# FedeMont/collision_handling_in_instantNGP

Measured on AMD Instinct MI355X. Metric: Mpixels/sec fwd+bwd at L=16,F=2,T=2^19, higher is better.
Workload: dtype f32

## Files before the change

collision_handling_in_instantngp_amd/_lib.py:

```python
import ctypes
import os

import torch

_HERE = os.path.dirname(os.path.abspath(__file__))
LIB_PATH = os.environ.get("GNGF_LIB_PATH") or os.path.join(_HERE, "libgngf_hip.so")

_c = ctypes
_P = _c.c_void_p
_I = _c.c_int
_L = _c.c_int64
_F = _c.c_float
_D = _c.c_double

SIGNATURES = {
    "gngf_abi_version": [],
    "gngf_hash_indices": [_P, _P, _P, _L, _I, _L, _P],
    "gngf_mrhe_fwd": [_P, _I, _P, _P, _P, _L, _I, _I, _L, _I, _I, _P],
    "gngf_mrhe_bwd": [_P, _I, _P, _P, _P, _P, _P, _L, _I, _I, _L, _I, _I, _P],
    "gngf_bilinear_fwd": [_P, _P, _P, _P, _L, _I, _I, _P],
    "gngf_bilinear_bwd": [_P, _P, _P, _P, _L, _I, _I, _P],
    "gngf_encode_fwd": [_P, _P, _I, _P, _P, _P, _P, _L, _I, _I, _L, _I, _I, _I, _L, _I, _I, _P, _P],
    "gngf_encode_bwd": [_P, _P, _I, _P, _P, _P, _P, _P, _P, _L, _I, _I, _L, _I, _I, _I, _L, _I, _I, _P],
    "gngf_encode_bwd_bucketed_plan": [_L, _I, _L, _I, _I, _P],
# ... 86 lines not shown
    "gngf_ext2_version": [],
    "gngf_ext2_render_score_workspace_words": [],
    "gngf_ext2_render_score": [_P, _I, _P, _P, _P, _P, _P, _P, _P, _P, _P, _I, _I, _L, _I, _I, _I, _L, _I, _I,
                               _P, _L, _L, _I, _F, _L, _P, _P, _P],
}

EXT2_VERSION = 1

_QUERY_TAIL = [_P, _L, _P, _P, _P]
EXT3_SIGNATURES = {
    "gngf_ext3_version": [],
    "gngf_ext3_query": [_P, _I, _P, _P, _P, _P, _P, _P, _P, _P, _P, _I, _I, _L, _I, _I, _I, _L, _I, _I] + _QUERY_TAIL,
    "gngf_ext3_query_grid": [_P, _P, _P, _P, _P, _P, _P, _P, _P, _I, _I, _I, _I] + _QUERY_TAIL,
    "gngf_ext3_vertex_grid_bwd_flat_owned": list(SIGNATURES["gngf_vertex_grid_bwd_flat"]),
    "gngf_ext3_encode_tiled_bwd_clear_rows": SIGNATURES["gngf_encode_tiled_bwd"][:-1] + [_P, _P, _I, _P],
}

EXT3_VERSION = 2

EXT3_WRITES_NOTHING = {
    "gngf_ext3_version": "returns a constant",
}


class BinJob(ctypes.Structure):
    _fields_ = [("xy", _P), ("P", _L), ("tile_shift", _I), ("NB", _I), ("chunk", _I), ("blockhist", _P), ("persistent_ws", _P),
                ("tile_off", _P), ("tile_item_base", _P), ("items", _P), ("n_items", _P), ("sorted", _P)]


_RETURNS_INT64 = {"gngf_decoder_hidden_floats", "gngf_slot_bitmap_words"}
_lib = None


class GngfLibraryError(RuntimeError):
    pass


def load():
    global _lib
    if _lib is not None:
        return _lib
    if not os.path.isfile(LIB_PATH):
        raise GngfLibraryError(
            f"{LIB_PATH} not found: build it with `python -c 'import __graft_entry__ as g; g.build()'` "
            "or `make -C collision_handling_in_instantngp_amd/csrc`.  There is no CPU fallback.")
    lib = ctypes.CDLL(LIB_PATH)
    for name, argtypes in (list(SIGNATURES.items()) + list(EXT_SIGNATURES.items()) + list(EXT2_SIGNATURES.items())
                           + list(EXT3_SIGNATURES.items())):
        try:
            fn = getattr(lib, name)
        except AttributeError as e:
            raise GngfLibraryError(f"{LIB_PATH} does not export {name}: stale build?") from e
        fn.argtypes = argtypes
        fn.restype = _L if name in _RETURNS_INT64 else _I
    ver = lib.gngf_abi_version()
    if ver != ABI_VERSION:
        raise GngfLibraryError(f"ABI version mismatch: library {ver}, binding {ABI_VERSION}")
    ext = lib.gngf_ext_version()
    if ext != EXT_VERSION:
        raise GngfLibraryError(f"extension version mismatch (include/gngf_ext.h): library {ext}, binding {EXT_VERSION}")
    ext2 = lib.gngf_ext2_version()
    if ext2 != EXT2_VERSION:
        raise GngfLibraryError(f"extension version mismatch (include/gngf_ext2.h): library {ext2}, binding {EXT2_VERSION}")
    ext3 = lib.gngf_ext3_version()
    if ext3 != EXT3_VERSION:
        raise GngfLibraryError(f"extension version mismatch (include/gngf_ext3.h): library {ext3}, binding {EXT3_VERSION}")
    _lib = lib
    return lib


def stream_ptr():
    return _P(torch.cuda.current_stream().cuda_stream)


def ptr(t, dtype=None, name="tensor"):
    if t is None:
        return _P(0)
    if not t.is_cuda:
        raise GngfLibraryError(f"{name} is on {t.device}: the gfx950 path needs CUDA/HIP tensors (no CPU fallback)")
    if dtype is not None and t.dtype != dtype:
        raise TypeError(f"{name} must be {dtype}, got {t.dtype}")
    if not t.is_contiguous():
        raise ValueError(f"{name} must be contiguous")
    return _P(t.data_ptr())


def query(name, *args):
    return getattr(load(), name)(*args)

# ... 17 lines not shown
```

collision_handling_in_instantngp_amd/csrc/decoder.hip:

```cpp
#include "gngf_common.h"
#include <type_traits>
#include <utility>

#include "decoder_common.inc"

namespace gngf {

__device__ __forceinline__ float vmax0(float z) { float r; asm("v_max_f32 %0, 0, %1" : "=v"(r) : "v"(z)); return r; }
template <bool LEAKY> __device__ __forceinline__ float hidden_act(float z) {
  if (LEAKY) { float r; const float t = 0.01f * z; asm("v_max_f32 %0, %1, %2" : "=v"(r) : "v"(z), "v"(t)); return r; }
  return vmax0(z);
}
template <bool LEAKY> __device__ __forceinline__ float hidden_dsel(float y, float d) { return y > 0.f ? d : (LEAKY ? 0.01f * d : 0.f); }

using f32x2 = __attribute__((ext_vector_type(2))) float;
__device__ __forceinline__ unsigned lds_addr(const float* p) {
  return (unsigned)(size_t)(__attribute__((address_space(3))) const float*)p;
}
template <int OFF> __device__ __forceinline__ void lds_store(unsigned addr, float v) {
  static_assert(OFF >= 0 && OFF < 65536, "ds offset is 16 bits");
  asm volatile("ds_write_b32 %0, %1 offset:%2" : : "v"(addr), "v"(v), "n"(OFF) : "memory");
}
template <int OFF> __device__ __forceinline__ f32x2 lds_load2(unsigned addr) {
  static_assert(OFF >= 0 && OFF < 65536, "ds offset is 16 bits");
// ... 29 lines not shown
  static constexpr int kA0 = 2 * S0 * 64, kA1 = 2 * 32 * 64, kA2 = 32 * 64;
};

template <int KIN>
__device__ __forceinline__ void fill_fwd_frags(float* A0, float* A1, const float* raw, int in_dim) {
  constexpr int S0 = KIN / 2;
  const RawOff o = raw_offsets(in_dim);
  for (int e = threadIdx.x; e < 2 * S0 * 64; e += kDecThreads) {
    const int lane = e & 63, s = (e >> 6) % S0, t = (e >> 6) / S0;
    const int i = lane & 31, h = lane >> 5, k = h * S0 + s;
    A0[e] = k < in_dim ? raw[o.w0 + (32 * t + i) * (in_dim + 1) + k] : 0.f;
  }
  for (int e = threadIdx.x; e < 2 * 32 * 64; e += kDecThreads) {
    const int lane = e & 63, s2 = (e >> 6) & 31, t = e >> 11;
    const int i = lane & 31, h = lane >> 5;
    A1[e] = raw[o.w1 + (32 * t + i) * 65 + kmapC(s2, h)];
  }
}

using u32x4 = __attribute__((ext_vector_type(4))) unsigned;

__device__ unsigned long long g_bwd_span[2];

#if defined(GNGF_STAMPS)
__device__ unsigned long long g_stamps[16];
__device__ unsigned long long g_fstamps[16];
__device__ unsigned long long g_blocktime[2][256][2];
#ifndef GNGF_STAMP_MASK
#define GNGF_STAMP_MASK 0xffff
#endif
#define STAMP(k) do { if constexpr ((((GNGF_STAMP_MASK) >> (k)) & 1) != 0) { unsigned long long t_; __builtin_amdgcn_sched_barrier(0); \
    asm volatile("s_memtime %0\n\ts_waitcnt lgkmcnt(0)" : "=s"(t_) :: "memory"); __builtin_amdgcn_sched_barrier(0); \
    ph[k] += t_ - tlast; tlast = t_; } } while (0)
#else
#define STAMP(k) do {} while (0)
#endif

constexpr int kHiddenTileFloats = 2 * 4 * 8 * 64 * 4;
#ifndef GNGF_BWD_X_AUX
#define GNGF_BWD_X_AUX 0
#endif
#ifndef GNGF_HIDDEN_AUX
#define GNGF_HIDDEN_AUX 2
#endif
#ifndef GNGF_HIDDEN_ST_AUX
#define GNGF_HIDDEN_ST_AUX GNGF_HIDDEN_AUX
// ... 173 lines not shown
    for (int k = 0; k < 10; ++k) g_fstamps[k] = ph[k];
  if (threadIdx.x == 0) g_blocktime[0][blockIdx.x & 255][1] = __builtin_readcyclecounter();
#endif
}

__host__ __device__ inline int slab_sums(int in_dim, int out_dim) { return kH * in_dim + kH * kH + out_dim * kH + 2 * kH + out_dim; }
__host__ __device__ inline int slab_size(int in_dim, int out_dim) { return slab_sums(in_dim, out_dim) + 1; }

constexpr int kImgStride = 34;
constexpr int kImgFloats = 64 * kImgStride;
#include "decoder_split.inc"
template <int KIN> struct BwdLds {
  static constexpr bool kDedicatedX = KIN <= 32;
  static constexpr int kWaveFloats = 2 * kImgFloats + 4 * kImgStride + (kDedicatedX ? KIN * kImgStride : 0);
};

template <int KIN, bool LEAKY, bool EXACT, bool RECOMPUTE, bool HYB = false, bool TRAIN = false>
__global__ void __launch_bounds__(kDecThreads, 1)
decoder_bwd_kernel(const float* __restrict__ X, const float* __restrict__ Yout, const float* __restrict__ dY,
                   const float* __restrict__ W0, const float* __restrict__ b0, const float* __restrict__ W1,
                   const float* __restrict__ b1, const float* __restrict__ W2, float* __restrict__ dX,
                   float* __restrict__ slabs, const float* __restrict__ hidden, int64_t P, int in_dim, int out_dim,
                   const float* __restrict__ target, const float* __restrict__ gloss, const float* __restrict__ b2 = nullptr,
                   float4* __restrict__ zero_fill = nullptr, int64_t zero_vecs = 0) {
  using FF = FwdFrags<KIN>;
  constexpr int S0 = KIN / 2;
  constexpr int TX = (KIN + 31) / 32;
  if (EXACT) in_dim = KIN;
  if (blockIdx.x == 0 && threadIdx.x == 0) { g_bwd_span[1] = 0ull; g_bwd_span[0] = wall_clock64(); }
#if defined(GNGF_STAMPS)
  if (threadIdx.x == 0) g_blocktime[1][blockIdx.x & 255][0] = __builtin_readcyclecounter();
#endif
  extern __shared__ float smem[];
  float* A0 = smem;
  float* A1 = A0 + FF::kA0;
  float* A2T = A1 + FF::kA1;
  static_assert(!HYB || (KIN == 32 && EXACT && !RECOMPUTE), "hybrid variant: 32 input features, saved hidden layers");
  static_assert(!TRAIN || HYB, "the fused training kernel builds on the hybrid backward");
  constexpr int kA1T = HYB ? 8 * 3 * 64 * 4 : 2 * 32 * 64, kA0T = HYB ? 4 * 3 * 64 * 4 : TX * 32 * 64;
  float* A1T = A2T + 2 * 2 * 64;
  float* A0T = A1T + kA1T;
  float* bs = A0T + kA0T;
  float* img = bs + 2 * kH;
  const int nslab = slab_size(in_dim, out_dim);

  float* raw = img;
  stage_raw(raw, W0, b0, W1, b1, W2, TRAIN ? b2 : nullptr, in_dim, out_dim);
// ... 134 lines not shown
    const __amdgpu_buffer_rsrc_t ry = __builtin_amdgcn_make_buffer_rsrc(const_cast<float*>(Yout) + tt * 128 * out_dim, 0, rows * out_dim * 4, 0x00020000);
    const __amdgpu_buffer_rsrc_t rd = __builtin_amdgcn_make_buffer_rsrc(const_cast<float*>(dsrc) + tt * 128 * out_dim, 0, rows * out_dim * 4, 0x00020000);
    if constexpr (TRAIN) {
#pragma unroll
      for (int sk = 0; sk < 2; ++sk) dyn[sk] = __uint_as_float(__builtin_amdgcn_raw_buffer_load_b32(rd, yoffh[sk], 0, 0));
    } else {
#pragma unroll
    for (int c = 0; c < 4; ++c) {
      const unsigned off = c < out_dim ? yoff + 4u * c : 0x40000000u;
      yn[c] = __uint_as_float(__builtin_amdgcn_raw_buffer_load_b32(ry, off, 0, 0));
      dyn[c] = __uint_as_float(__builtin_amdgcn_raw_buffer_load_b32(rd, off, 0, 0));
    }
    }
  };
  auto make_dz3 = [&]() {
#pragma unroll
    for (int c = 0; c < (TRAIN ? 2 : 4); ++c) {
      const float dy = fused_loss ? kloss * (yn[c] - dyn[c]) : dyn[c];
      dz3[c] = dy * (yn[c] * (1.f - yn[c]));
      asm volatile("" : "+v"(dz3[c]));
      db2acc[c] += dz3[c];
    }
  };
  fetch_x(blockIdx.x);
  fetch_y(blockIdx.x);
  if constexpr (!TRAIN) make_dz3();
  float b2v[4] = {0.f, 0.f, 0.f, 0.f};
  if constexpr (TRAIN) {
#pragma unroll
    for (int sk = 0; sk < 2; ++sk) b2v[sk] = raw[ro.b2 + 2 * sk + h];
  }
  f32x16 b0v[2], b1v[2];
  if (RECOMPUTE) {
#pragma unroll
    for (int t = 0; t < 2; ++t) {
#pragma unroll
      for (int r = 0; r < 16; ++r) { b0v[t][r] = bs[32 * t + crow(r, h)]; b1v[t][r] = bs[kH + 32 * t + crow(r, h)]; }
      asm volatile("" : "+a"(b0v[t]), "+a"(b1v[t]));
    }
  }
  unsigned dxmax = 0u;
#if defined(GNGF_STAMPS)
  unsigned ph[16] = {0, 0, 0, 0, 0, 0, 0, 0, 0, 0, 0, 0, 0, 0, 0, 0};
  unsigned long long tlast;
  asm volatile("s_memtime %0\n\ts_waitcnt lgkmcnt(0)" : "=s"(tlast) :: "memory");
#endif
// ... 20 lines not shown
  };
  if constexpr (HYB && !TRAIN) static_for<16>([&](auto E) { store_hidden_images(E); });
  const u32x4* w1t = reinterpret_cast<const u32x4*>(A1T) + lane;
  const u32x4* w0t = reinterpret_cast<const u32x4*>(A0T) + lane;
  Planes w1p[HYB ? 8 : 1], w0p[HYB ? 4 : 1];
  if constexpr (HYB) {
#pragma unroll
    for (int f = 0; f < 8; ++f) {
      w1p[f] = load_planes(w1t + f * 3 * 64);
      asm volatile("" : "+a"(w1p[f].hi), "+a"(w1p[f].mid), "+a"(w1p[f].lo));
    }
  }
  u32x4* w1f = reinterpret_cast<u32x4*>(A1T);
  if constexpr (TRAIN) {
    asm volatile("s_waitcnt lgkmcnt(0)" ::: "memory");
    __syncthreads();
    for (int f = threadIdx.x >> 6; f < 8; f += 4) {
      const int cc = f >> 1, t = f & 1;
      const float* r1 = raw + ro.w1 + (32 * t + i) * 65;
      store_planes(w1f + f * 3 * 64 + lane, split8(r1[kmapS(cc, h, 0)], r1[kmapS(cc, h, 1)], r1[kmapS(cc, h, 2)], r1[kmapS(cc, h, 3)],
                                                  r1[kmapS(cc, h, 4)], r1[kmapS(cc, h, 5)], r1[kmapS(cc, h, 6)], r1[kmapS(cc, h, 7)]));
    }
    __syncthreads();
  }
  if (RECOMPUTE && kCarryF0) {
#pragma unroll
    for (int sx = 0; sx < S0; ++sx) { f0[0][sx] = A0[(0 * S0 + sx) * 64 + lane]; f0[1][sx] = A0[(1 * S0 + sx) * 64 + lane]; }
  }
#define STEP_END() __builtin_amdgcn_sched_barrier(0)
#define SLOT_END() __builtin_amdgcn_sched_barrier(0)
#define SLOT_END1(x) do { asm volatile("" : "+a"(x)); __builtin_amdgcn_sched_barrier(0); } while (0)
#define SLOT_END2(x, y) do { asm volatile("" : "+a"(x), "+a"(y)); __builtin_amdgcn_sched_barrier(0); } while (0)
  for (int64_t tile = blockIdx.x; tile < ntiles; tile += gridDim.x) {
    pin_acc();
    STAMP(0);
    float f1[2][32];
    float a2t[2][2];
    if constexpr (TRAIN) {
      Planes pa0 = load_planes(w0f + lane), pa1 = load_planes(w0f + 3 * 64 + lane);
#pragma unroll
      for (int t = 0; t < 2; ++t)
#pragma unroll
        for (int g = 0; g < 4; ++g) {
          const f32x4 q0 = *reinterpret_cast<const f32x4*>(bs + 32 * t + 8 * g + 4 * h);
          const f32x4 q1 = *reinterpret_cast<const f32x4*>(bs + kH + 32 * t + 8 * g + 4 * h);
#pragma unroll
          for (int e = 0; e < 4; ++e) { acc1[t][4 * g + e] = q0[e]; acc2[t][4 * g + e] = q1[e]; }
        }
      Planes zc = split8(xr[0], xr[1], xr[2], xr[3], xr[4], xr[5], xr[6], xr[7]);
      STAMP(8);
      unsigned nh[4], nm[4], nl[4];
      float sra, srb;
      auto next_planes = [&]() {
        Planes p;
        p.hi = u32x4{nh[0], nh[1], nh[2], nh[3]}; p.mid = u32x4{nm[0], nm[1], nm[2], nm[3]}; p.lo = u32x4{nl[0], nl[1], nl[2], nl[3]};
        return p;
      };
// ... 165 lines not shown
        if constexpr (TRAIN) {
          fa[0][sk] = a2t[0][sk]; fa[1][sk] = a2t[1][sk];
          bsel[sk] = dz3[sk];
        } else {
        fa[0][sk] = A2T[(0 * 2 + sk) * 64 + lane]; fa[1][sk] = A2T[(1 * 2 + sk) * 64 + lane];
        float lo = dz3[2 * sk], hi = dz3[2 * sk + 1];
        asm volatile("" : "+v"(lo), "+v"(hi));
        bsel[sk] = h == 0 ? lo : hi;
        }
      }
      STEP_END();
      MFMA_VV_ZERO(d2[0], fa[0][0], bsel[0]); MFMA_VV_ZERO(d2[1], fa[1][0], bsel[0]);
      MFMA_VV(d2[0], fa[0][1], bsel[1]); MFMA_VV(d2[1], fa[1][1], bsel[1]);
      if constexpr (TRAIN) {
        asm volatile("" : "+v"(d2[0]), "+v"(d2[1]));
        STEP_END();
      }
      if constexpr (!RECOMPUTE) {
        if (BL::kDedicatedX) static_for<S0>([&](auto SX) { lds_store<kImgX + SX.value * kImgStride * 4>(wX, xr[SX.value]); });
        if constexpr (TRAIN) static_for<2>([&](auto SK) { lds_store<kImgZ + 2 * SK.value * kImgStride * 4>(wDz3h, dz3[SK.value]); });
        else static_for<4>([&](auto C) { lds_store<kImgZ + C.value * kImgStride * 4>(wDz3, dz3[C.value]); });
      }
    }
    if (!RECOMPUTE && BL::kDedicatedX) fetch_x(tile + gridDim.x);
    fetch_y(tile + gridDim.x);
    MFMA_DRAIN(d2[0], d2[1]);
    STEP_END();
    STAMP(12);
    if constexpr (TRAIN) {
#pragma unroll
      for (int r = 0; r < 8; ++r) d2[0][r] = hidden_dsel<LEAKY>(acc2[0][r], d2[0][r]);
    } else {
#pragma unroll
    for (int t = 0; t < 2; ++t)
#pragma unroll
      for (int r = 0; r < 16; ++r) {
        if (RECOMPUTE) acc2[t][r] = hidden_act<LEAKY>(acc2[t][r]);
        d2[t][r] = hidden_dsel<LEAKY>(acc2[t][r], d2[t][r]);
      }
    }
    pin_acc();
    STEP_END();
    STAMP(3);
    f32x16 d1[2];
    f32x2 a0p[8], a1p[8], b0p[8], b1p[8];
    float h1v[2][16];
    if constexpr (HYB) {
      f32x2 av[16], bv[16];
// ... 355 lines not shown
          const int col = 32 * tx + 8 * g + 4 * h;
          if (EXACT) {
            if (32 * tx + 8 * g + 8 <= KIN) {
              u32x4 v = {__float_as_uint(dxv[tx][4 * g]), __float_as_uint(dxv[tx][4 * g + 1]), __float_as_uint(dxv[tx][4 * g + 2]),
                         __float_as_uint(dxv[tx][4 * g + 3])};
              __builtin_amdgcn_raw_buffer_store_b128(v, rs, base + 4u * col, 0, 0);
            }
          } else {
#pragma unroll
            for (int q = 0; q < 4; ++q)
              __builtin_amdgcn_raw_buffer_store_b32(__float_as_uint(dxv[tx][4 * g + q]), rs, col + q < in_dim ? base + 4u * (col + q) : 0x40000000u, 0, 0);
          }
        }
    }
    if constexpr (kClears) {
      for (int z = 0; z < zper; ++z, zlo += kDecThreads)
        if (zlo < zhi) zero_fill[zlo] = float4{0.f, 0.f, 0.f, 0.f};
    }
    pin_acc();
    STEP_END();
    STAMP(7);
  }

#if defined(GNGF_STAMPS)
  if (blockIdx.x == 7 && threadIdx.x == 0)
    for (int k = 0; k < 16; ++k) g_stamps[k] = ph[k];
  if (threadIdx.x == 0) g_blocktime[1][blockIdx.x & 255][1] = __builtin_readcyclecounter();
#endif
#pragma unroll
  for (int o = 32; o > 0; o >>= 1) { const unsigned ov = (unsigned)__shfl_xor((int)dxmax, o, 64); dxmax = ov > dxmax ? ov : dxmax; }
  __syncthreads();
  float* region = smem + wave * nslab;
  float* sW0 = region;
  float* sW1 = sW0 + kH * in_dim;
  float* sW2 = sW1 + kH * kH;
  float* sb0 = sW2 + out_dim * kH;
  float* sb1 = sb0 + kH;
  float* sb2 = sb1 + kH;
#pragma unroll
  for (int ti = 0; ti < 2; ++ti)
#pragma unroll
    for (int r = 0; r < 16; ++r) {
      const int row = 32 * ti + crow(r, h);
#pragma unroll
      for (int tj = 0; tj < 2; ++tj) sW1[row * kH + 32 * tj + i] = dW1acc[ti][tj][r];
#pragma unroll
// ... 117 lines not shown
  GNGF_CHECK_ARG(slabs && (!reduce_here || (dW0 && db0 && dW1 && db1 && dW2 && db2)));
  const int nslab = slab_size(in_dim, out_dim);
  hipStream_t s = as_stream(stream);
  const int nslabs = gngf_decoder_bwd_slabs(P);
  if (P == 0) {
    hipError_t e = zero_async(slabs, sizeof(float) * (size_t)nslab, s);
    if (e != hipSuccess) return (int)e;
    if (zero_fill && zero_floats > 0) {
      e = zero_async(zero_fill, sizeof(float) * (size_t)zero_floats, s);
      if (e != hipSuccess) return (int)e;
    }
  } else {
    GNGF_CHECK_ARG(enc && rgb && (target ? gloss != nullptr : drgb != nullptr) && W0 && b0 && W1 && b1 && W2 && denc);
    if (zero_fill && zero_floats > 0 && in_dim != 64) {
      hipError_t e = zero_async(zero_fill, sizeof(float) * (size_t)zero_floats, s);
      if (e != hipSuccess) return (int)e;
    }
    if (g_decoder_bwd_hybrid && in_dim == 32 && hidden) {
      const size_t smem = bwd_smem_bytes_hybrid(out_dim);
      auto fn = leaky ? decoder_bwd_kernel<32, true, true, false, true> : decoder_bwd_kernel<32, false, true, false, true>;
      hipError_t e = hipFuncSetAttribute(reinterpret_cast<const void*>(fn), hipFuncAttributeMaxDynamicSharedMemorySize, (int)smem);
      if (e != hipSuccess) return (int)e;
      fn<<<dim3((unsigned)nslabs), dim3(kDecThreads), smem, s>>>(enc, rgb, drgb, W0, b0, W1, b1, W2, denc, slabs, hidden, P, in_dim, out_dim,
                                                                 target, gloss, nullptr, zf, zv);
    } else
    DISPATCH_KIN(in_dim, {
      const size_t smem = bwd_smem_bytes<kKIN>(in_dim, out_dim);
      using Kern = void (*)(const float*, const float*, const float*, const float*, const float*, const float*, const float*,
                            const float*, float*, float*, const float*, int64_t, int, int, const float*, const float*, const float*,
                            float4*, int64_t);
      const bool exact = in_dim == kKIN;
      Kern fn;
      if (hidden)
        fn = leaky ? (exact ? decoder_bwd_kernel<kKIN, true, true, false> : decoder_bwd_kernel<kKIN, true, false, false>)
                   : (exact ? decoder_bwd_kernel<kKIN, false, true, false> : decoder_bwd_kernel<kKIN, false, false, false>);
      else
        fn = leaky ? (exact ? decoder_bwd_kernel<kKIN, true, true, true> : decoder_bwd_kernel<kKIN, true, false, true>)
                   : (exact ? decoder_bwd_kernel<kKIN, false, true, true> : decoder_bwd_kernel<kKIN, false, false, true>);
      hipError_t e = hipFuncSetAttribute(reinterpret_cast<const void*>(fn), hipFuncAttributeMaxDynamicSharedMemorySize, (int)smem);
      if (e != hipSuccess) return (int)e;
      fn<<<dim3((unsigned)nslabs), dim3(kDecThreads), smem, s>>>(enc, rgb, drgb, W0, b0, W1, b1, W2, denc, slabs, hidden, P, in_dim, out_dim,
                                                                 target, gloss, nullptr, zf, zv);
    });
    hipError_t e = hipGetLastError();
    if (e != hipSuccess) return (int)e;
  }
  if (reduce_here)
    decoder_reduce_kernel<<<dim3((unsigned)((nslab + 63) / 64)), dim3(1024), 0, s>>>(slabs, nslabs, nslab, in_dim, out_dim, dW0,
                                                                                     db0, dW1, db1, dW2, db2, denc_absmax, nullptr, nullptr);
  GNGF_RETURN_LAUNCH();
}

extern "C" int gngf_decoder_train(const float* enc, const float* target, const float* gloss, const float* W0, const float* b0,
                                  const float* W1, const float* b1, const float* W2, const float* b2, float* rgb, float* denc,
                                  float* dW0, float* db0, float* dW1, float* db1, float* dW2, float* db2, float* slabs,
                                  float* denc_absmax, float* zero_fill, int64_t zero_floats, int64_t P, int in_dim, int out_dim,
                                  int leaky, void* stream) {
  GNGF_CHECK_ARG(P > 0 && in_dim == 32 && out_dim > 0 && out_dim <= 4);
  GNGF_CHECK_ARG(!zero_fill || (zero_floats >= 0 && (zero_floats & 3) == 0 && (reinterpret_cast<uintptr_t>(zero_fill) & 15) == 0));
  const bool reduce_here = dW0 || db0 || dW1 || db1 || dW2 || db2;
  GNGF_CHECK_ARG(slabs && (!reduce_here || (dW0 && db0 && dW1 && db1 && dW2 && db2)));
  GNGF_CHECK_ARG(enc && target && gloss && W0 && b0 && W1 && b1 && W2 && b2 && rgb && denc);
  const int nslab = slab_size(in_dim, out_dim);
  hipStream_t s = as_stream(stream);
  const int nslabs = gngf_decoder_bwd_slabs(P);
  const size_t smem = bwd_smem_bytes_hybrid(out_dim);
  auto fn = leaky ? decoder_bwd_kernel<32, true, true, false, true, true> : decoder_bwd_kernel<32, false, true, false, true, true>;
  hipError_t e = hipFuncSetAttribute(reinterpret_cast<const void*>(fn), hipFuncAttributeMaxDynamicSharedMemorySize, (int)smem);
  if (e != hipSuccess) return (int)e;
  fn<<<dim3((unsigned)nslabs), dim3(kDecThreads), smem, s>>>(enc, rgb, nullptr, W0, b0, W1, b1, W2, denc, slabs, nullptr, P, in_dim, out_dim,
                                                             target, gloss, b2, reinterpret_cast<float4*>(zero_fill),
                                                             zero_fill ? zero_floats / 4 : 0);
  e = hipGetLastError();
  if (e != hipSuccess) return (int)e;
  if (reduce_here)
    decoder_reduce_kernel<<<dim3((unsigned)((nslab + 63) / 64)), dim3(1024), 0, s>>>(slabs, nslabs, nslab, in_dim, out_dim, dW0,
                                                                                     db0, dW1, db1, dW2, db2, denc_absmax, nullptr, nullptr);
  GNGF_RETURN_LAUNCH();
}

extern "C" int gngf_decoder_reduce(const float* slabs, float* dW0, float* db0, float* dW1, float* db1, float* dW2, float* db2,
                                   float* denc_absmax, const float* gloss_promised, const float* gloss_arrived, int64_t P,
                                   int in_dim, int out_dim, void* stream) {
  GNGF_CHECK_ARG(P >= 0 && in_dim > 0 && in_dim <= 64 && out_dim > 0 && out_dim <= 4);
  GNGF_CHECK_ARG(slabs && dW0 && db0 && dW1 && db1 && dW2 && db2 && (!gloss_promised == !gloss_arrived));
  const int nslab = slab_size(in_dim, out_dim);
  decoder_reduce_kernel<<<dim3((unsigned)((nslab + 63) / 64)), dim3(1024), 0, as_stream(stream)>>>(
      slabs, gngf_decoder_bwd_slabs(P), nslab, in_dim, out_dim, dW0, db0, dW1, db1, dW2, db2, denc_absmax, gloss_promised,
      gloss_arrived);
  GNGF_RETURN_LAUNCH();
}

extern "C" int gngf_decoder_bwd_last_span_ns(double* ns) {
  GNGF_CHECK_ARG(ns);
  unsigned long long span[2] = {0ull, 0ull};
  hipError_t e = hipMemcpyFromSymbol(span, HIP_SYMBOL(gngf::g_bwd_span), sizeof(span));
  if (e != hipSuccess) return (int)e;
  *ns = span[1] > span[0] ? (double)(span[1] - span[0]) * 10.0 : 0.0;
  return 0;
}

#if defined(GNGF_STAMPS)
extern "C" int gngf_debug_read_fwd_stamps(unsigned long long* host16) {
  return (int)hipMemcpyFromSymbol(host16, HIP_SYMBOL(gngf::g_fstamps), 16 * sizeof(unsigned long long));
}
extern "C" int gngf_debug_read_blocktime(unsigned long long* host1024) {
  return (int)hipMemcpyFromSymbol(host1024, HIP_SYMBOL(gngf::g_blocktime), 2 * 256 * 2 * sizeof(unsigned long long));
}
extern "C" int gngf_debug_read_stamps(unsigned long long* host16) {
  return (int)hipMemcpyFromSymbol(host16, HIP_SYMBOL(gngf::g_stamps), 16 * sizeof(unsigned long long));
}
#endif

#include "render.inc"
```

collision_handling_in_instantngp_amd/ops.py:

```python
import ctypes as _ct
import dataclasses as _dc
import math as _math
import os
import sys as _sys
import types as _types

import torch

from . import _lib
from ._lib import call, ptr, query, stream_ptr

BLEND_CODES = {True: 0, None: 1, False: 2}
MODE_HASH, MODE_VERTEX_TABLE = 0, 1
MODE_DENSE_HASH = 2
MAX_TOPK = 128
MAX_TOPK_LIST = 32


def check_topk(K):
    K = int(K)
    if K > MAX_TOPK:
        raise ValueError(f"topk_k = {K} exceeds the limit of {MAX_TOPK} (ops.MAX_TOPK, GNGF_MAX_TOPK_WIDE)")
    return K

# ... 1268 lines not shown
    if not TUNING.use_side_stream:
        return torch.cuda.current_stream(device)
    key = (device.type, device.index, torch.cuda.current_stream(device).stream_id)
    if key not in _SIDE_STREAMS:
        _SIDE_STREAMS[key] = torch.cuda.Stream(device=device)
    return _SIDE_STREAMS[key]


@_dc.dataclass(frozen=True)
class StepConfig:
    source: str
    staged: int
    direct: int
    binning: str
    vertex_fwd: str
    pixel: str
    grad_sink: str
    table_grad: str
    clear: str
    direct_bwd: str
    exchange: bool
    vertex_bwd_flat: bool = False
    owned_rows: bool = False

    def signature(self):
        return (f"{self.source} L{self.staged}+{self.direct} bin={self.binning} vfwd={self.vertex_fwd} px={self.pixel} sink={self.grad_sink} "
                f"dE={self.table_grad}/{self.clear} direct={self.direct_bwd}" + (" xchg" if self.exchange else "")
                + (" vbwd=flat" if self.vertex_bwd_flat else "") + (" rows=owned" if self.owned_rows else ""))

    def chain(self):
        lv = ("tiled" if self.staged else "") + ("+" if self.staged and self.direct else "") + ("direct" if self.direct else "")
        return (f"{self.source} {lv} bin={self.binning} vfwd={self.vertex_fwd} px={self.pixel} sink={self.grad_sink} "
                f"dE={self.table_grad}/{self.clear} direct={self.direct_bwd}" + (" xchg" if self.exchange else ""))

    @staticmethod
    def choose(plan, L, T, F, P, mode, fp32_tables, needs_grad, link_defer_zero, link_zero_hidden, exchange, persist_ok, persist_alloc_ok,
               have_reserve_ws, flat_list=False, owned_rows=False):
        t = TUNING
        tiled = plan.Ls > 0 and P > 0
        nd = L - plan.Ls
        if mode == MODE_DENSE_HASH:
            if exchange:
                raise ValueError("the dense-where-it-fits index source does not run under a data-parallel exchange")
            dbw = "atomics" if (needs_grad and nd > 0) else "none"
            if not tiled:
                return StepConfig("dense_hash", 0, L, "none", "none", "none", "none", "alloc" if needs_grad else "none", "none", dbw, False)
            il = plan.interleaved(backward=bool(needs_grad))
            if not needs_grad:
                return StepConfig("dense_hash", plan.Ls, nd, "prepare", "riders", "interleaved" if il else "generic", "none", "none", "none",
                                  "none", False)
# ... 51 lines not shown
        K = check_topk(0 if vert_idx is None else vert_idx.shape[1])
        NV = 0 if vert_idx is None else vert_idx.shape[0]
        enc = torch.empty((P, L * F), dtype=_f32, device=tables.device)
        ws = None
        ctx.flat = (_flat_list_of(order, plan, vert_idx, vert_w, T)
                    if (P > 0 and ctx.needs_input_grad[3] and not ctx.needs_input_grad[5]) else None)
        if vert_idx is not None and order is None and plan.Ls > 0 and P > 0 and ctx.needs_input_grad[3]:
            order = slot_order(vert_idx, plan.n_ls_host[:plan.Ls], vstride)
        buf = None
        clear_now = None
        dev = tables.device
        tiled = plan.Ls > 0 and P > 0
        pws = _bin_workspace(dev, plan.ntiles, dp, kind="reserve") if (tiled and TUNING.fused_vertex_fwd) else None
        choose_args = (
            plan, L, T, F, P, mode, tables.dtype == _f32, bool(ctx.needs_input_grad[3]),
            bool(link is not None and link.defer_zero), bool(link is not None and link.zero_hidden),
            bool(dp is not None and dp.exchange is not None), bool(dp is not None and dp.persist_ok and getattr(dp, "level_params", None)),
            bool(dp is not None and (getattr(dp, "persist_grad", None) is not None or not torch.cuda.is_current_stream_capturing())),
            bool(pws is not None and pws.numel() >= 2 * plan.ntiles + 3))
        want_owned = bool(VERTEX_BWD_OWNED and ctx.flat is not None
                          and StepConfig.choose(*choose_args, flat_list=True, owned_rows=True).owned_rows)
        sc = ctx.step_config = StepConfig.choose(*choose_args, flat_list=ctx.flat is not None,
                                                 owned_rows=want_owned and _owned_peek(dp, tables, ctx.flat) is not None)
        if dp is not None:
            dp.step_config = sc
        _trace("step_config", signature=sc.signature())
        if SEEN_STEP_CONFIGS is not None:
            SEEN_STEP_CONFIGS.add(sc.chain())
        if tiled:
            fused = sc.vertex_fwd == "fused" and sc.binning == "pipeline"
            use64 = sc.grad_sink == "dG64"
            if ctx.needs_input_grad[3]:
                ng = 0 if sc.grad_sink == "table_rows" else ((plan.vtot * F + 2) * 2 if use64 else plan.vtot * F)
                nt = tables.numel()
                if fused and sc.owned_rows:
                    big = torch.empty(((ng + 3) & ~3,), dtype=_f32, device=dev)
                    buf = _BackwardBuffers(big[:ng].view(_i64), None, zbuf=big, owned=True)
                elif fused:
                    big = torch.empty((nt + ((ng + 3) & ~3),), dtype=_f32, device=dev)
                    dgrid = None if ng == 0 else (big[nt:nt + ng].view(_i64) if use64 else big[nt:nt + ng].view(plan.vtot, F))
                    buf = _BackwardBuffers(dgrid, big[:nt].view(tables.shape), zbuf=big)
                else:
                    dgrid = None if ng == 0 else (torch.empty((plan.vtot * F + 2,), dtype=_i64, device=dev) if use64
                                                  else torch.empty((plan.vtot, F), dtype=_f32, device=dev))
                    if sc.table_grad == "persist":
                        clear_now = _persistent_peek(dp, tables)
# ... 443 lines not shown
        return
    call("gngf_ext3_query", *pointers, *scalars, ptr(xy, _f32, "xy"), P, ptr(out_rgb, _f32, "out_rgb"),
         ptr(out_image, _i32, "out_image"), stream_ptr())


def query_grid_points(grid, n_ls, n_ls_host, decoder_params, xy, *, leaky=False, out_rgb=None, out_image=None):
    C, pointers, scalars = _grid_model("query_grid_points", grid, n_ls, n_ls_host, decoder_params, leaky)
    P = _query_tail("query_grid_points", xy, C, out_rgb, out_image)
    if P == 0:
        return
    call("gngf_ext3_query_grid", *pointers, *scalars, ptr(xy, _f32, "xy"), P, ptr(out_rgb, _f32, "out_rgb"),
         ptr(out_image, _i32, "out_image"), stream_ptr())



def _at_end_of_backward(fn):
    try:
        torch.autograd.Variable._execution_engine.queue_callback(fn)
    except RuntimeError:
        fn()


_GLOSS_SCALARS = {}


def _decoder_grad_buffers(ws, P, in_dim, out_dim, dev):
    flat = torch.empty((sum(w.numel() for w in ws),), dtype=_f32, device=dev)
    grads, off = [], 0
    for w in ws:
        grads.append(flat[off:off + w.numel()].view(w.shape))
        off += w.numel()
    nslabs, nslab = _lib.query("gngf_decoder_bwd_slabs", P), _lib.query("gngf_decoder_slab_floats", in_dim, out_dim)
    slabs = torch.empty((nslabs * nslab,), dtype=_f32, device=dev)
    return flat, grads, slabs, nslabs, nslab


def _decoder_fwd(ctx, enc, leaky, ws, target, gloss_known=None, link=None):
    ctx.ws_given = tuple(ws)
    ctx.link = link = link if link is not None else StepLink()
    enc = _c(enc)
    ws = [_c(w) for w in ws]
    P, in_dim = enc.shape
    out_dim = ws[4].shape[0]
    dev = enc.device
    rgb = torch.empty((P, out_dim), dtype=_f32, device=dev)
    hidden = None
    ctx.train = None
    train = (TUNING.decoder_train_fusion and gloss_known is not None and target is not None and in_dim == 32 and P > 0
             and TUNING.decoder_reduce_rides and any(ctx.needs_input_grad))
    if TUNING.decoder_save_hidden and P > 0 and any(ctx.needs_input_grad) and not train:
        hidden = torch.empty((_lib.query("gngf_decoder_hidden_floats", P),), dtype=_f32, device=dev)
    if target is not None:
        if P == 0:
            raise ValueError("MSE of an empty batch")
        target = _c(target)
        if tuple(target.shape) != (P, out_dim) or target.dtype != _f32:
            raise ValueError(f"target {tuple(target.shape)} / {target.dtype} does not match the decoder output ({P}, {out_dim}) float32")
    if train:
        key = (dev, float(gloss_known))
        gl = _GLOSS_SCALARS.get(key)
        if gl is None:
            if len(_GLOSS_SCALARS) > 64:
                _GLOSS_SCALARS.clear()
            gl = _GLOSS_SCALARS[key] = torch.full((), float(gloss_known), dtype=_f32, device=dev)
        target_c = _c(target)
        denc = torch.empty_like(enc)
        flat, grads, slabs, nslabs, nslab = _decoder_grad_buffers(ws, P, in_dim, out_dim, dev)
        zr, link.zero_request = link.zero_request, None
        call("gngf_decoder_train", ptr(enc, _f32, "enc"), ptr(target_c, _f32, "target"), ptr(gl), *[ptr(w, _f32) for w in ws], ptr(rgb),
             ptr(denc), *[ptr(None)] * 6, ptr(slabs), ptr(None), ptr(zr), 0 if zr is None else zr.numel(), P, in_dim, out_dim,
             int(leaky), stream_ptr())
        ctx.train = {"denc": denc, "flat": flat, "grads": grads, "slabs": slabs, "nslabs": nslabs, "nslab": nslab,
                     "gloss": float(gloss_known), "promised": gl}
    else:
        call("gngf_decoder_fwd", ptr(enc, _f32, "enc"), *[ptr(w, _f32) for w in ws], ptr(rgb), ptr(hidden), P, in_dim, out_dim, int(leaky),
             stream_ptr())
    mse = None
    if target is not None:
        wsp = _MSE_WORKSPACE.get(dev)
        if wsp is None:
            wsp = _MSE_WORKSPACE[dev] = torch.zeros(query("gngf_mse_workspace_floats"), dtype=_f32, device=dev)
        mse = torch.empty((), dtype=_f32, device=dev)
        if link.loss_value_aside:
            link.loss_value = {"pred": rgb, "label": target, "loss": mse, "ws": wsp, "device": dev,
                               "stream": torch.cuda.current_stream(dev).cuda_stream, "stream_obj": torch.cuda.current_stream(dev)}
        else:
            call("gngf_mse_fwd", ptr(rgb), ptr(target), ptr(mse), ptr(wsp), rgb.numel(), stream_ptr())
    ctx.save_for_backward(enc, rgb, target, *ws)
    ctx.hidden = hidden
    ctx.cfg = (P, in_dim, out_dim, int(leaky))
    return rgb, mse


def _grads_are_adopted(ctx):
# ... 160 lines not shown
```

Measured before the change: 2738.

## Add per-wave stagger option and incremental next-tile prefetch in decoder train kernel

Adds an optional per-wave sleep stagger after the prologue of the fused decoder train kernel, exposed through a new ext4 entry point, with a default of zero so the default path runs no sleeps. It also replaces the per-tile fetch_x/fetch_y prefetch in the forward (train) path with an incremental window pointer that advances by gridDim and builds buffer resources sized to the remaining rows. That is meant to cut 64-bit address arithmetic on each tile. A debug wave-phase timestamp probe is added behind a compile flag.

```diff
diff --git a/collision_handling_in_instantngp_amd/_lib.py b/collision_handling_in_instantngp_amd/_lib.py
--- a/collision_handling_in_instantngp_amd/_lib.py
+++ b/collision_handling_in_instantngp_amd/_lib.py
@@ -132,6 +132,28 @@
     "gngf_ext3_version": "returns a constant",
 }
 
+_U64 = ctypes.c_uint64
+EXT4_SIGNATURES = {
+    "gngf_ext4_version": [],
+    "gngf_ext4_decoder_train_default_stagger": [],
+    "gngf_ext4_decoder_train": SIGNATURES["gngf_decoder_train"][:-1] + [_U64, _P],
+}
+
+EXT4_VERSION = 1
+MAX_STAGGER_UNITS = 1023
+DEFAULT_DECODER_TRAIN_STAGGER = 0
+
+
+def stagger_pattern(l0, l1, l2, l3):
+    lags = (int(l0), int(l1), int(l2), int(l3))
+    if any(l < 0 or l > 0xffff for l in lags):
+        raise ValueError(f"stagger lags are 16-bit fields: {lags}")
+    return lags[0] | lags[1] << 16 | lags[2] << 32 | lags[3] << 48
+
+
+def stagger_lags(pattern):
+    return tuple((int(pattern) >> (16 * w)) & 0xffff for w in range(4))
+
 
 class BinJob(ctypes.Structure):
     _fields_ = [("xy", _P), ("P", _L), ("tile_shift", _I), ("NB", _I), ("chunk", _I), ("blockhist", _P), ("persistent_ws", _P),
@@ -139,6 +161,7 @@
 
 
 _RETURNS_INT64 = {"gngf_decoder_hidden_floats", "gngf_slot_bitmap_words"}
+_RETURNS_UINT64 = {"gngf_ext4_decoder_train_default_stagger"}
 _lib = None
 
 
@@ -156,13 +179,13 @@
             "or `make -C collision_handling_in_instantngp_amd/csrc`.  There is no CPU fallback.")
     lib = ctypes.CDLL(LIB_PATH)
     for name, argtypes in (list(SIGNATURES.items()) + list(EXT_SIGNATURES.items()) + list(EXT2_SIGNATURES.items())
-                           + list(EXT3_SIGNATURES.items())):
+                           + list(EXT3_SIGNATURES.items()) + list(EXT4_SIGNATURES.items())):
         try:
             fn = getattr(lib, name)
         except AttributeError as e:
             raise GngfLibraryError(f"{LIB_PATH} does not export {name}: stale build?") from e
         fn.argtypes = argtypes
-        fn.restype = _L if name in _RETURNS_INT64 else _I
+        fn.restype = _L if name in _RETURNS_INT64 else (_U64 if name in _RETURNS_UINT64 else _I)
     ver = lib.gngf_abi_version()
     if ver != ABI_VERSION:
         raise GngfLibraryError(f"ABI version mismatch: library {ver}, binding {ABI_VERSION}")
@@ -175,6 +198,13 @@
     ext3 = lib.gngf_ext3_version()
     if ext3 != EXT3_VERSION:
         raise GngfLibraryError(f"extension version mismatch (include/gngf_ext3.h): library {ext3}, binding {EXT3_VERSION}")
+    ext4 = lib.gngf_ext4_version()
+    if ext4 != EXT4_VERSION:
+        raise GngfLibraryError(f"extension version mismatch (include/gngf_ext4.h): library {ext4}, binding {EXT4_VERSION}")
+    stagger = lib.gngf_ext4_decoder_train_default_stagger()
+    if stagger != DEFAULT_DECODER_TRAIN_STAGGER:
+        raise GngfLibraryError(f"default stagger pattern mismatch (include/gngf_ext4.h): library {stagger:#x}, "
+                               f"binding {DEFAULT_DECODER_TRAIN_STAGGER:#x}")
     _lib = lib
     return lib
 
diff --git a/collision_handling_in_instantngp_amd/csrc/decoder.hip b/collision_handling_in_instantngp_amd/csrc/decoder.hip
--- a/collision_handling_in_instantngp_amd/csrc/decoder.hip
+++ b/collision_handling_in_instantngp_amd/csrc/decoder.hip
@@ -1,4 +1,5 @@
 #include "gngf_common.h"
+#include "../../include/gngf_ext4.h"
 #include <type_traits>
 #include <utility>
 
@@ -75,6 +76,10 @@
 
 __device__ unsigned long long g_bwd_span[2];
 
+#if defined(GNGF_WAVE_PHASE)
+constexpr int kPhaseTiles[5] = {0, 1, 8, 16, 31};
+__device__ unsigned g_wave_phase[4][4][5];
+#endif
 #if defined(GNGF_STAMPS)
 __device__ unsigned long long g_stamps[16];
 __device__ unsigned long long g_fstamps[16];
@@ -294,7 +299,7 @@
                    const float* __restrict__ b1, const float* __restrict__ W2, float* __restrict__ dX,
                    float* __restrict__ slabs, const float* __restrict__ hidden, int64_t P, int in_dim, int out_dim,
                    const float* __restrict__ target, const float* __restrict__ gloss, const float* __restrict__ b2 = nullptr,
-                   float4* __restrict__ zero_fill = nullptr, int64_t zero_vecs = 0) {
+                   float4* __restrict__ zero_fill = nullptr, int64_t zero_vecs = 0, unsigned long long stagger = 0ull) {
   using FF = FwdFrags<KIN>;
   constexpr int S0 = KIN / 2;
   constexpr int TX = (KIN + 31) / 32;
@@ -475,6 +480,24 @@
       db2acc[c] += dz3[c];
     }
   };
+  constexpr bool kStepWindow = TRAIN && !GNGF_BWD_REVERSE;
+  auto fetch_next = [&](unsigned gdim, int& nwin, const float*& wx, const float*& wd) {
+    nwin += (int)gdim;
+    wx += gdim * 128u * (unsigned)in_dim;
+    wd += gdim * 128u * (unsigned)out_dim;
+    const int last_tile = (int)(ntiles - 1);
+    const int rows = nwin < last_tile ? 128 : (nwin == last_tile ? (int)(P - (ntiles - 1) * 128) : 0);
+    const __amdgpu_buffer_rsrc_t rx = __builtin_amdgcn_make_buffer_rsrc(const_cast<float*>(wx), 0, rows * in_dim * 4, 0x00020000);
+    const __amdgpu_buffer_rsrc_t rd = __builtin_amdgcn_make_buffer_rsrc(const_cast<float*>(wd), 0, rows * out_dim * 4, 0x00020000);
+#pragma unroll
+    for (int k = 0; k < S0 / 4; ++k) {
+      const u32x4 v = __builtin_amdgcn_raw_buffer_load_b128(rx, xoff + 16 * k, 0, GNGF_BWD_X_AUX);
+      xr[4 * k] = __uint_as_float(v.x); xr[4 * k + 1] = __uint_as_float(v.y);
+      xr[4 * k + 2] = __uint_as_float(v.z); xr[4 * k + 3] = __uint_as_float(v.w);
+    }
+#pragma unroll
+    for (int sk = 0; sk < 2; ++sk) dyn[sk] = __uint_as_float(__builtin_amdgcn_raw_buffer_load_b32(rd, yoffh[sk], 0, 0));
+  };
   fetch_x(blockIdx.x);
   fetch_y(blockIdx.x);
   if constexpr (!TRAIN) make_dz3();
@@ -541,6 +564,8 @@
                                                   r1[kmapS(cc, h, 4)], r1[kmapS(cc, h, 5)], r1[kmapS(cc, h, 6)], r1[kmapS(cc, h, 7)]));
     }
     __syncthreads();
+    for (unsigned n = __builtin_amdgcn_readfirstlane((unsigned)(stagger >> (16 * wave)) & 0xffffu); n != 0u; --n)
+      __builtin_amdgcn_s_sleep(1);
   }
   if (RECOMPUTE && kCarryF0) {
 #pragma unroll
@@ -550,8 +575,30 @@
 #define SLOT_END() __builtin_amdgcn_sched_barrier(0)
 #define SLOT_END1(x) do { asm volatile("" : "+a"(x)); __builtin_amdgcn_sched_barrier(0); } while (0)
 #define SLOT_END2(x, y) do { asm volatile("" : "+a"(x), "+a"(y)); __builtin_amdgcn_sched_barrier(0); } while (0)
+#if defined(GNGF_WAVE_PHASE)
+  unsigned wphase[5] = {0u, 0u, 0u, 0u, 0u}, wpass = 0u;
+#endif
+  [[maybe_unused]] unsigned gdim = 0u;
+  [[maybe_unused]] int nwin = 0;
+  [[maybe_unused]] const float *wx = nullptr, *wd = nullptr;
+  if constexpr (kStepWindow) {
+    gdim = gridDim.x;
+    asm volatile("" : "+s"(gdim));
+    nwin = (int)blockIdx.x;
+    wx = X + (int64_t)blockIdx.x * 128 * in_dim;
+    wd = dsrc + (int64_t)blockIdx.x * 128 * out_dim;
+  }
   for (int64_t tile = blockIdx.x; tile < ntiles; tile += gridDim.x) {
     pin_acc();
+#if defined(GNGF_WAVE_PHASE)
+    if constexpr (TRAIN) {
+      unsigned long long t_;
+      asm volatile("s_memtime %0\n\ts_waitcnt lgkmcnt(0)" : "=s"(t_) :: "memory");
+#pragma unroll
+      for (int k = 0; k < 5; ++k) wphase[k] = wpass == (unsigned)kPhaseTiles[k] ? (unsigned)t_ : wphase[k];
+      ++wpass;
+    }
+#endif
     STAMP(0);
     float f1[2][32];
     float a2t[2][2];
@@ -763,8 +810,11 @@
         else static_for<4>([&](auto C) { lds_store<kImgZ + C.value * kImgStride * 4>(wDz3, dz3[C.value]); });
       }
     }
+    if constexpr (kStepWindow) fetch_next(gdim, nwin, wx, wd);
+    else {
     if (!RECOMPUTE && BL::kDedicatedX) fetch_x(tile + gridDim.x);
     fetch_y(tile + gridDim.x);
+    }
     MFMA_DRAIN(d2[0], d2[1]);
     STEP_END();
     STAMP(12);
@@ -1166,6 +1216,10 @@
     STAMP(7);
   }
 
+#if defined(GNGF_WAVE_PHASE)
+  if (TRAIN && blockIdx.x < 4 && (threadIdx.x & 63) == 0)
+    for (int k = 0; k < 5; ++k) g_wave_phase[blockIdx.x][threadIdx.x >> 6][k] = wphase[k];
+#endif
 #if defined(GNGF_STAMPS)
   if (blockIdx.x == 7 && threadIdx.x == 0)
     for (int k = 0; k < 16; ++k) g_stamps[k] = ph[k];
@@ -1329,13 +1383,13 @@
       hipError_t e = hipFuncSetAttribute(reinterpret_cast<const void*>(fn), hipFuncAttributeMaxDynamicSharedMemorySize, (int)smem);
       if (e != hipSuccess) return (int)e;
       fn<<<dim3((unsigned)nslabs), dim3(kDecThreads), smem, s>>>(enc, rgb, drgb, W0, b0, W1, b1, W2, denc, slabs, hidden, P, in_dim, out_dim,
-                                                                 target, gloss, nullptr, zf, zv);
+                                                                 target, gloss, nullptr, zf, zv, 0ull);
     } else
     DISPATCH_KIN(in_dim, {
       const size_t smem = bwd_smem_bytes<kKIN>(in_dim, out_dim);
       using Kern = void (*)(const float*, const float*, const float*, const float*, const float*, const float*, const float*,
                             const float*, float*, float*, const float*, int64_t, int, int, const float*, const float*, const float*,
-                            float4*, int64_t);
+                            float4*, int64_t, unsigned long long);
       const bool exact = in_dim == kKIN;
       Kern fn;
       if (hidden)
@@ -1347,7 +1401,7 @@
       hipError_t e = hipFuncSetAttribute(reinterpret_cast<const void*>(fn), hipFuncAttributeMaxDynamicSharedMemorySize, (int)smem);
       if (e != hipSuccess) return (int)e;
       fn<<<dim3((unsigned)nslabs), dim3(kDecThreads), smem, s>>>(enc, rgb, drgb, W0, b0, W1, b1, W2, denc, slabs, hidden, P, in_dim, out_dim,
-                                                                 target, gloss, nullptr, zf, zv);
+                                                                 target, gloss, nullptr, zf, zv, 0ull);
     });
     hipError_t e = hipGetLastError();
     if (e != hipSuccess) return (int)e;
@@ -1358,12 +1412,14 @@
   GNGF_RETURN_LAUNCH();
 }
 
-extern "C" int gngf_decoder_train(const float* enc, const float* target, const float* gloss, const float* W0, const float* b0,
-                                  const float* W1, const float* b1, const float* W2, const float* b2, float* rgb, float* denc,
-                                  float* dW0, float* db0, float* dW1, float* db1, float* dW2, float* db2, float* slabs,
-                                  float* denc_absmax, float* zero_fill, int64_t zero_floats, int64_t P, int in_dim, int out_dim,
-                                  int leaky, void* stream) {
+static int decoder_train_launch(const float* enc, const float* target, const float* gloss, const float* W0, const float* b0,
+                                const float* W1, const float* b1, const float* W2, const float* b2, float* rgb, float* denc,
+                                float* dW0, float* db0, float* dW1, float* db1, float* dW2, float* db2, float* slabs,
+                                float* denc_absmax, float* zero_fill, int64_t zero_floats, int64_t P, int in_dim, int out_dim,
+                                int leaky, uint64_t stagger, void* stream) {
   GNGF_CHECK_ARG(P > 0 && in_dim == 32 && out_dim > 0 && out_dim <= 4);
+  GNGF_CHECK_ARG(P < ((int64_t)1 << 37));
+  for (int w = 0; w < 4; ++w) GNGF_CHECK_ARG(((stagger >> (16 * w)) & 0xffffu) <= (uint64_t)GNGF_EXT4_MAX_STAGGER_UNITS);
   GNGF_CHECK_ARG(!zero_fill || (zero_floats >= 0 && (zero_floats & 3) == 0 && (reinterpret_cast<uintptr_t>(zero_fill) & 15) == 0));
   const bool reduce_here = dW0 || db0 || dW1 || db1 || dW2 || db2;
   GNGF_CHECK_ARG(slabs && (!reduce_here || (dW0 && db0 && dW1 && db1 && dW2 && db2)));
@@ -1377,13 +1433,33 @@
   if (e != hipSuccess) return (int)e;
   fn<<<dim3((unsigned)nslabs), dim3(kDecThreads), smem, s>>>(enc, rgb, nullptr, W0, b0, W1, b1, W2, denc, slabs, nullptr, P, in_dim, out_dim,
                                                              target, gloss, b2, reinterpret_cast<float4*>(zero_fill),
-                                                             zero_fill ? zero_floats / 4 : 0);
+                                                             zero_fill ? zero_floats / 4 : 0, (unsigned long long)stagger);
   e = hipGetLastError();
   if (e != hipSuccess) return (int)e;
   if (reduce_here)
     decoder_reduce_kernel<<<dim3((unsigned)((nslab + 63) / 64)), dim3(1024), 0, s>>>(slabs, nslabs, nslab, in_dim, out_dim, dW0,
                                                                                      db0, dW1, db1, dW2, db2, denc_absmax, nullptr, nullptr);
   GNGF_RETURN_LAUNCH();
+}
+
+extern "C" int gngf_decoder_train(const float* enc, const float* target, const float* gloss, const float* W0, const float* b0,
+                                  const float* W1, const float* b1, const float* W2, const float* b2, float* rgb, float* denc,
+                                  float* dW0, float* db0, float* dW1, float* db1, float* dW2, float* db2, float* slabs,
+                                  float* denc_absmax, float* zero_fill, int64_t zero_floats, int64_t P, int in_dim, int out_dim,
+                                  int leaky, void* stream) {
+  return decoder_train_launch(enc, target, gloss, W0, b0, W1, b1, W2, b2, rgb, denc, dW0, db0, dW1, db1, dW2, db2, slabs, denc_absmax,
+                              zero_fill, zero_floats, P, in_dim, out_dim, leaky, GNGF_EXT4_DEFAULT_STAGGER, stream);
+}
+
+extern "C" int gngf_ext4_version(void) { return GNGF_EXT4_VERSION; }
+extern "C" uint64_t gngf_ext4_decoder_train_default_stagger(void) { return GNGF_EXT4_DEFAULT_STAGGER; }
+extern "C" int gngf_ext4_decoder_train(const float* enc, const float* target, const float* gloss, const float* W0, const float* b0,
+                                       const float* W1, const float* b1, const float* W2, const float* b2, float* rgb, float* denc,
+                                       float* dW0, float* db0, float* dW1, float* db1, float* dW2, float* db2, float* slabs,
+                                       float* denc_absmax, float* zero_fill, int64_t zero_floats, int64_t P, int in_dim,
+                                       int out_dim, int leaky, uint64_t stagger, void* stream) {
+  return decoder_train_launch(enc, target, gloss, W0, b0, W1, b1, W2, b2, rgb, denc, dW0, db0, dW1, db1, dW2, db2, slabs, denc_absmax,
+                              zero_fill, zero_floats, P, in_dim, out_dim, leaky, stagger, stream);
 }
 
 extern "C" int gngf_decoder_reduce(const float* slabs, float* dW0, float* db0, float* dW1, float* db1, float* dW2, float* db2,
@@ -1407,6 +1483,11 @@
   return 0;
 }
 
+#if defined(GNGF_WAVE_PHASE)
+extern "C" int gngf_debug_read_wave_phase(unsigned* host80) {
+  return (int)hipMemcpyFromSymbol(host80, HIP_SYMBOL(gngf::g_wave_phase), 4 * 4 * 5 * sizeof(unsigned));
+}
+#endif
 #if defined(GNGF_STAMPS)
 extern "C" int gngf_debug_read_fwd_stamps(unsigned long long* host16) {
   return (int)hipMemcpyFromSymbol(host16, HIP_SYMBOL(gngf::g_fstamps), 16 * sizeof(unsigned long long));
diff --git a/collision_handling_in_instantngp_amd/ops.py b/collision_handling_in_instantngp_amd/ops.py
--- a/collision_handling_in_instantngp_amd/ops.py
+++ b/collision_handling_in_instantngp_amd/ops.py
@@ -1314,10 +1314,12 @@
     exchange: bool
     vertex_bwd_flat: bool = False
     owned_rows: bool = False
+    stagger: int = 0
 
     def signature(self):
         return (f"{self.source} L{self.staged}+{self.direct} bin={self.binning} vfwd={self.vertex_fwd} px={self.pixel} sink={self.grad_sink} "
                 f"dE={self.table_grad}/{self.clear} direct={self.direct_bwd}" + (" xchg" if self.exchange else "")
+                + (" stagger=" + "/".join(str(l) for l in _lib.stagger_lags(self.stagger)) if self.stagger else "")
                 + (" vbwd=flat" if self.vertex_bwd_flat else "") + (" rows=owned" if self.owned_rows else ""))
 
     def chain(self):
@@ -1415,6 +1417,8 @@
                           and StepConfig.choose(*choose_args, flat_list=True, owned_rows=True).owned_rows)
         sc = ctx.step_config = StepConfig.choose(*choose_args, flat_list=ctx.flat is not None,
                                                  owned_rows=want_owned and _owned_peek(dp, tables, ctx.flat) is not None)
+        if link is not None and link.zero_hidden and DECODER_TRAIN_STAGGER:
+            sc = ctx.step_config = _dc.replace(sc, stagger=int(DECODER_TRAIN_STAGGER))
         if dp is not None:
             dp.step_config = sc
         _trace("step_config", signature=sc.signature())
@@ -1904,6 +1908,7 @@
 
 
 _GLOSS_SCALARS = {}
+DECODER_TRAIN_STAGGER = _lib.DEFAULT_DECODER_TRAIN_STAGGER
 
 
 def _decoder_grad_buffers(ws, P, in_dim, out_dim, dev):
@@ -1949,9 +1954,11 @@
         denc = torch.empty_like(enc)
         flat, grads, slabs, nslabs, nslab = _decoder_grad_buffers(ws, P, in_dim, out_dim, dev)
         zr, link.zero_request = link.zero_request, None
-        call("gngf_decoder_train", ptr(enc, _f32, "enc"), ptr(target_c, _f32, "target"), ptr(gl), *[ptr(w, _f32) for w in ws], ptr(rgb),
-             ptr(denc), *[ptr(None)] * 6, ptr(slabs), ptr(None), ptr(zr), 0 if zr is None else zr.numel(), P, in_dim, out_dim,
-             int(leaky), stream_ptr())
+        stagger = int(DECODER_TRAIN_STAGGER)
+        own = stagger != _lib.DEFAULT_DECODER_TRAIN_STAGGER
+        call("gngf_ext4_decoder_train" if own else "gngf_decoder_train", ptr(enc, _f32, "enc"), ptr(target_c, _f32, "target"), ptr(gl),
+             *[ptr(w, _f32) for w in ws], ptr(rgb), ptr(denc), *[ptr(None)] * 6, ptr(slabs), ptr(None), ptr(zr),
+             0 if zr is None else zr.numel(), P, in_dim, out_dim, int(leaky), *([stagger] if own else []), stream_ptr())
         ctx.train = {"denc": denc, "flat": flat, "grads": grads, "slabs": slabs, "nslabs": nslabs, "nslab": nslab,
                      "gloss": float(gloss_known), "promised": gl}
     else:
diff --git a/include/gngf_ext4.h b/include/gngf_ext4.h
--- /dev/null
+++ b/include/gngf_ext4.h
@@ -0,0 +1,31 @@
+#ifndef GNGF_EXT4_H_
+#define GNGF_EXT4_H_
+
+#include <stdint.h>
+
+#ifdef __cplusplus
+extern "C" {
+#endif
+
+#define GNGF_EXT4_VERSION 1
+
+int gngf_ext4_version(void);
+
+#define GNGF_EXT4_MAX_STAGGER_UNITS 1023
+#define GNGF_EXT4_STAGGER(l0, l1, l2, l3) \
+  ((uint64_t)(l0) | ((uint64_t)(l1) << 16) | ((uint64_t)(l2) << 32) | ((uint64_t)(l3) << 48))
+#define GNGF_EXT4_DEFAULT_STAGGER GNGF_EXT4_STAGGER(0, 0, 0, 0)
+
+uint64_t gngf_ext4_decoder_train_default_stagger(void);
+
+int gngf_ext4_decoder_train(const float* enc, const float* target, const float* gloss, const float* W0, const float* b0,
+                            const float* W1, const float* b1, const float* W2, const float* b2, float* rgb, float* denc,
+                            float* dW0, float* db0, float* dW1, float* db1, float* dW2, float* db2, float* slabs,
+                            float* denc_absmax, float* zero_fill, int64_t zero_floats, int64_t P, int in_dim, int out_dim,
+                            int leaky, uint64_t stagger, void* stream);
+
+#ifdef __cplusplus
+}
+#endif
+
+#endif
```

Measured after the change: 2726. No clear change (-0.4%).
